# RuihanGao/visual-tactile-synthesis

Hardware: AMD Instinct MI355X
Metric: train_images_per_sec (higher is better)
Workload: dtype f32; 1 GPU; skitG G+D1+D2 train step, 1024x1024 sketch->(RGB,tactile), 4 images/GPU, 64 tactile patches/image, LPIPS/CLIP terms off (no weights offline); global_batch=4, parallelism=dp1, losses_finite=True, hip_graph=True, d2_visualisation_pass=True, train_only=False, full=False

## Files before the change

visual-tactile-synthesis_amd/csrc/vts_conv_head.hip:

```cpp
#include <limits.h>
#include <stdlib.h>

#include "vts_internal.h"

namespace {

struct HeadK {
  const float* x;
  const float *sc, *sh;
  int64_t ns;
  int C, IH, IW, OH, OW, pad, padx;
  const float* w;
  int ws_ci;
  const float* bias;
  float* out;
  int64_t ons;
  float slope;
  const float* ident;
};

constexpr int HK_TY = 32, HK_TX = 32, HK_PR = HK_TY + 3, HK_PC = HK_TX + 3, HK_PCP = 36;
constexpr int HK_MAXC = 512;

template <int CK>
__global__ __launch_bounds__(1024) void conv_head_kernel(const HeadK p) {
  constexpr int BLOCK = 1024, NG = BLOCK / 256, CPG = CK / NG;
  static_assert(CK % NG == 0, "a chunk splits evenly over the thread groups");
  constexpr int NEL = CK * HK_PR * HK_PC;
  constexpr int NLD = (NEL + BLOCK - 1) / BLOCK;
  __shared__ __attribute__((aligned(16))) float tile[CK][HK_PR][HK_PCP];
  __shared__ __attribute__((aligned(16))) float wl[CK][16];
  __shared__ float ssc[HK_MAXC], ssh[HK_MAXC];
  const int tid = threadIdx.x, n = blockIdx.z;
  const int grp = __builtin_amdgcn_readfirstlane(tid >> 8), t256 = tid & 255;
  const int tx4 = t256 & 7, ty = t256 >> 3;
  const int oy0 = blockIdx.y * HK_TY, ox0 = blockIdx.x * HK_TX;
  const int iy0 = oy0 - p.pad, ix0 = ox0 - p.padx;
  for (int c = tid; c < p.C; c += BLOCK) {
    ssc[c] = p.sc ? p.sc[n * p.C + c] : 1.f;
    ssh[c] = p.sh ? p.sh[n * p.C + c] : 0.f;
  }
  int soff[NLD], sdst[NLD];
  const int64_t plane = (int64_t)p.IH * p.IW;
#pragma unroll
  for (int i = 0; i < NLD; ++i) {
    const int e = i * BLOCK + tid;
    const int c = e / (HK_PR * HK_PC), rem = e - c * (HK_PR * HK_PC);
    const int r = rem / HK_PC, col = rem - r * HK_PC;
    const int iy = iy0 + r, ix = ix0 + col;
    const bool in = e < NEL && iy >= 0 && iy < p.IH && ix >= 0 && ix < p.IW;
    soff[i] = in ? iy * p.IW + ix : -1;
    sdst[i] = e < NEL ? (c * HK_PR + r) * HK_PCP + col : -1;
  }
  const float* xb = p.x + n * p.ns;
  float pv[NLD];
  static_assert(BLOCK <= HK_PR * HK_PC, "one boundary per slot");
  auto chan = [&](int i) {
    const int b = (i * BLOCK) / (HK_PR * HK_PC);
    return b + (tid >= (b + 1) * (HK_PR * HK_PC) - i * BLOCK ? 1 : 0);
  };
  auto load_chunk = [&](int c0) {
#pragma unroll
    for (int i = 0; i < NLD; ++i) {
      const int c = c0 + chan(i);
      pv[i] = (soff[i] >= 0 && c < p.C) ? xb[c * plane + soff[i]] : 0.f;
    }
  };
  auto store_chunk = [&](int c0) {
    float* t = &tile[0][0][0];
#pragma unroll
    for (int i = 0; i < NLD; ++i) {
      const int c = c0 + chan(i);
      if (sdst[i] >= 0) {
        const bool ok = soff[i] >= 0 && c < p.C;
        const int cc = min(c, p.C - 1);
        const float u = fmaf(pv[i], ssc[cc], ssh[cc]);
        t[sdst[i]] = ok ? fmaxf(u, 0.f) + p.slope * fminf(u, 0.f) : 0.f;
      }
    }
    if (tid < CK * 16) {
      const int c = c0 + (tid >> 4);
      wl[tid >> 4][tid & 15] = c < p.C ? p.w[(int64_t)c * p.ws_ci + (tid & 15)] : 0.f;
    }
  };
  float acc[4] = {0.f, 0.f, 0.f, 0.f};
  __syncthreads();
  load_chunk(0);
  store_chunk(0);
  __syncthreads();
  for (int c0 = 0; c0 < p.C; c0 += CK) {
    const bool more = c0 + CK < p.C;
    if (more) load_chunk(c0 + CK);
#pragma unroll
    for (int cg = 0; cg < CPG; ++cg) {
      const int c = grp * CPG + cg;
#pragma unroll
      for (int ky = 0; ky < 4; ++ky) {
        const f32x4 a = *reinterpret_cast<const f32x4*>(&tile[c][ty + ky][tx4 * 4]);
        const f32x4 b = *reinterpret_cast<const f32x4*>(&tile[c][ty + ky][tx4 * 4 + 4]);
        const f32x4 wv = *reinterpret_cast<const f32x4*>(&wl[c][ky * 4]);
        const float v[8] = {a[0], a[1], a[2], a[3], b[0], b[1], b[2], b[3]};
#pragma unroll
        for (int kx = 0; kx < 4; ++kx)
#pragma unroll
          for (int j = 0; j < 4; ++j) acc[j] = fmaf(v[j + kx], wv[kx], acc[j]);
      }
    }
    __syncthreads();
    if (more) {
      store_chunk(c0 + CK);
      __syncthreads();
    }
  }
  f32x4* red = reinterpret_cast<f32x4*>(&tile[0][0][0]);
  if (grp > 0) red[(grp - 1) * 256 + t256] = (f32x4){acc[0], acc[1], acc[2], acc[3]};
  __syncthreads();
  if (grp > 0) return;
#pragma unroll
  for (int g = 1; g < NG; ++g) {
    const f32x4 v = red[(g - 1) * 256 + t256];
#pragma unroll
    for (int j = 0; j < 4; ++j) acc[j] += v[j];
  }
  const float bias = p.bias ? p.bias[0] : 0.f;
  const int y = oy0 + ty;
  if (y < p.OH) {
    float* o = p.out + n * p.ons + (int64_t)y * p.OW;
#pragma unroll
    for (int j = 0; j < 4; ++j) {
      const int x = ox0 + tx4 * 4 + j;
      if (x < p.OW) o[x] = acc[j] + bias;
    }
  }
}

struct HeadSK {
  const float* x;
  const float *sc, *sh;
  int64_t ns;
  int C, N, IH, IW, OH, OW, pad, padx;
  const float* w;
  int ws_ci;
  const float* bias;
  float* out;
  int64_t ons;
  float slope;
  int IPB, PH, PW, CK;
};

__global__ __launch_bounds__(256) void conv_head_small_kernel(const HeadSK p) {
  extern __shared__ __attribute__((aligned(16))) float smem[];
  float* tile = smem;
  float* wl = smem + p.IPB * p.CK * p.PH * p.PW;
  const int tid = threadIdx.x;
  const int n0 = blockIdx.x * p.IPB;
  const int nimg = min(p.IPB, p.N - n0);
  const int plane = p.PH * p.PW, ohw = p.OH * p.OW, ihw = p.IH * p.IW;
  const int img = tid / ohw, r = tid - img * ohw;
  const int oy = r / p.OW, ox = r - oy * p.OW;
  const bool active = img < nimg;
  const int base = img * p.CK * plane + oy * p.PW + ox;
  for (int i = tid; i < p.IPB * p.CK * plane; i += 256) tile[i] = 0.f;
  float acc = 0.f;
  for (int c0 = 0; c0 < p.C; c0 += p.CK) {
    __syncthreads();
    const int total = nimg * p.CK * ihw;
    for (int e0 = tid; e0 < total; e0 += 256 * 8) {
      float raw[8], fsc[8], fsh[8];
      int dst[8];
#pragma unroll
      for (int j = 0; j < 8; ++j) {
        const int e = e0 + j * 256;
        const int ee = min(e, total - 1);
        const int ic = ee / ihw, q = ee - ic * ihw;
        const int im = ic / p.CK, c = ic - im * p.CK;
        const int y = q / p.IW, x = q - y * p.IW;
        const int cc = min(c0 + c, p.C - 1), n = n0 + im;
        raw[j] = p.x[n * p.ns + (int64_t)cc * ihw + q];
        fsc[j] = p.sc ? p.sc[n * p.C + cc] : 1.f;
        fsh[j] = p.sh ? p.sh[n * p.C + cc] : 0.f;
        dst[j] = (e < total && c0 + c < p.C) ? (im * p.CK + c) * plane + (y + p.pad) * p.PW + x + p.padx : -1 - ((im * p.CK + c) * plane + (y + p.pad) * p.PW + x + p.padx);
        if (e >= total) dst[j] = INT_MIN;
      }
#pragma unroll
      for (int j = 0; j < 8; ++j) {
        const float t = fmaf(raw[j], fsc[j], fsh[j]);
        if (dst[j] >= 0) tile[dst[j]] = fmaxf(t, 0.f) + p.slope * fminf(t, 0.f);
        else if (dst[j] != INT_MIN) tile[-1 - dst[j]] = 0.f;
      }
    }
    for (int e = tid; e < p.CK * 16; e += 256) wl[e] = (c0 + (e >> 4) < p.C) ? p.w[(int64_t)(c0 + (e >> 4)) * p.ws_ci + (e & 15)] : 0.f;
    __syncthreads();
    if (active) {
#pragma unroll 4
      for (int c = 0; c < p.CK; ++c) {
        const float* t = tile + base + c * plane;
#pragma unroll
        for (int ky = 0; ky < 4; ++ky)
#pragma unroll
          for (int kx = 0; kx < 4; ++kx) acc = fmaf(t[ky * p.PW + kx], wl[c * 16 + ky * 4 + kx], acc);
      }
    }
  }
  if (active) p.out[(n0 + img) * p.ons + r] = acc + (p.bias ? p.bias[0] : 0.f);
}

}

int vts_conv_head_try(const vts_conv_desc* d, hipStream_t st) {
  if (d->transposed || d->stride != 1 || d->Cout != 1 || d->in1.data || d->dmask.data || d->accumulate || d->act_out != VTS_ACT_NONE)
    return VTS_ERR_UNSUPPORTED;
  if (d->in0.C > HK_MAXC || d->in0.C < 8 || (int64_t)d->IH * d->IW * d->in0.C >= (1ll << 31)) return VTS_ERR_UNSUPPORTED;
  if ((int64_t)d->OH * d->OW < 1024) {
    const int padx = d->pad + d->pad_dx;
    if (d->N < 32 || d->OH * d->OW > 256 || d->pad < 0 || padx < 0 || d->IH + d->pad < d->OH + 3 - d->pad || d->IW + padx < d->OW + 3 - padx)
      return VTS_ERR_UNSUPPORTED;
    HeadSK q;
    q.x = d->in0.data; q.sc = d->in0.scale; q.sh = d->in0.shift; q.ns = d->in0.nstride; q.C = d->in0.C; q.N = d->N;
    q.IH = d->IH; q.IW = d->IW; q.OH = d->OH; q.OW = d->OW; q.pad = d->pad; q.padx = padx;
    q.w = d->w; q.ws_ci = d->ws_ci; q.bias = d->bias; q.out = d->out; q.ons = d->out_nstride; q.slope = vts_slope(d->act_in);
    q.PH = d->IH + 2 * d->pad; q.PW = d->IW + 2 * padx;
    q.IPB = 256 / (d->OH * d->OW);
    q.CK = d->in0.C;
    auto bytes = [&]() { return (int64_t)(q.IPB * q.CK * q.PH * q.PW + q.CK * 16) * 4; };
    while (q.IPB > 2 && bytes() > 60 * 1024) --q.IPB;
    if (bytes() > 60 * 1024) {
      q.CK = 16;
      q.IPB = 256 / (d->OH * d->OW);
      while (q.IPB > 1 && bytes() > 60 * 1024) --q.IPB;
    }
    const int lds = (int)bytes();
    if (lds > 64 * 1024) return VTS_ERR_UNSUPPORTED;
    hipLaunchKernelGGL(conv_head_small_kernel, dim3(cdiv(d->N, q.IPB)), dim3(256), lds, st, q);
    vts_set_kernel("conv_head_small_kernel");
    VTS_CHECK_LAUNCH("vts_conv4x4 (head, small maps)");
    return VTS_OK;
  }
  HeadK k;
  k.x = d->in0.data; k.sc = d->in0.scale; k.sh = d->in0.shift; k.ns = d->in0.nstride; k.C = d->in0.C;
  k.IH = d->IH; k.IW = d->IW; k.OH = d->OH; k.OW = d->OW; k.pad = d->pad; k.padx = d->pad + d->pad_dx;
  k.w = d->w; k.ws_ci = d->ws_ci; k.bias = d->bias; k.out = d->out; k.ons = d->out_nstride;
  k.slope = vts_slope(d->act_in);
  k.ident = nullptr;
  dim3 grid(cdiv(d->OW, HK_TX), cdiv(d->OH, HK_TY), d->N);
  hipLaunchKernelGGL((conv_head_kernel<8>), grid, dim3(1024), 0, st, k);
  vts_set_kernel("conv_head_kernel<8>");
  VTS_CHECK_LAUNCH("vts_conv4x4 (head)");
  return VTS_OK;
}
```

visual-tactile-synthesis_amd/csrc/vts_wgrad.hip:

```cpp
#include <stdio.h>
#include <stdlib.h>

#include "vts_internal.h"

namespace {

struct Src {
  const float *d0, *d1, *sc0, *sh0, *sc1, *sh1;
  int64_t ns0, ns1;
  int C0, C1, C;
  int act;
  float slope;
  const float* ident;
  int plain;
};

struct WgK {
  Src lo, hi;
  int N, LH, LW, HH, HW, pad, padx;
  int cl_groups, ch_groups;
  int tiles_y, tiles_x, ntiles;
  float* part;
  int ablate;
};
// ... 672 lines not shown
          for (int t = 0; t < CLT; ++t)
#pragma unroll
            for (int c = 0; c < CHW; ++c) acc[t][c] = __builtin_amdgcn_mfma_f32_16x16x4f32(a[u][t], b[u][c], acc[t][c], 0, 0, 0);
        }
      }
    }
    __syncthreads();
  }
  float* part = p.part + (int64_t)blockIdx.x * p.CL * p.CH * 16;
#pragma unroll
  for (int t = 0; t < CLT; ++t)
#pragma unroll
    for (int c = 0; c < CHW; ++c) {
      const int ch = wave * CHW + c;
#pragma unroll
      for (int r = 0; r < 4; ++r) {
        const int cl = t * 16 + kq * 4 + r;
        if (cl < p.CL && ch < p.CH) part[((int64_t)cl * p.CH + ch) * 16 + m16] = acc[t][c][r];
      }
    }
}

struct HeadWK {
  const float* lo;
  int64_t lons;
  const float *hi, *hisc, *hish;
  int64_t hins;
  int CH, N, LH, LW, HH, HW, pad, padx;
  float hi_slope;
  int tiles_y, tiles_x;
  float* part;
};
constexpr int HWG_TY = 16, HWG_TX = 32, HWG_PR = HWG_TY + 3, HWG_PC = HWG_TX + 3, HWG_PCP = 36, HWG_CK = 16, HWG_PLANE = HWG_PR * HWG_PCP;

__global__ __launch_bounds__(256) void wgrad_head_kernel(const HeadWK p) {
  __shared__ __attribute__((aligned(16))) float patch[HWG_CK * HWG_PLANE];
  __shared__ __attribute__((aligned(16))) float dyt[HWG_TY * HWG_PCP];
  const int tid = threadIdx.x;
  const int tile = blockIdx.x;
  const int n = tile / (p.tiles_y * p.tiles_x), rem = tile - n * (p.tiles_y * p.tiles_x);
  const int ty = rem / p.tiles_x, tx = rem - ty * p.tiles_x;
  const int y0 = ty * HWG_TY, x0 = tx * HWG_TX;
  const int hy0 = y0 - p.pad, hx0 = x0 - p.padx;
  for (int e = tid; e < HWG_TY * HWG_TX; e += 256) {
    const int r = e >> 5, c = e & 31;
    const int y = y0 + r, x = x0 + c;
    dyt[r * HWG_PCP + c] = (y < p.LH && x < p.LW) ? p.lo[n * p.lons + (int64_t)y * p.LW + x] : 0.f;
  }
  const int rg = tid & 3, ky = (tid >> 2) & 3, chl = tid >> 4;
  const int64_t hplane = (int64_t)p.HH * p.HW;
  float* part = p.part + (int64_t)tile * p.CH * 16;
  const int lane = tid & 63;
  const int wv = __builtin_amdgcn_readfirstlane(tid >> 6);
  const int ix = hx0 + lane;
  const bool colok = lane < HWG_PC && ix >= 0 && ix < p.HW;
  const int ixc = min(max(ix, 0), p.HW - 1);
  float raw[HWG_CK / 4][HWG_PR];
  auto load_chunk = [&](int c0) {
#pragma unroll
    for (int cc = 0; cc < HWG_CK / 4; ++cc) {
      const int chc = min(c0 + wv + 4 * cc, p.CH - 1);
      const float* src = p.hi + n * p.hins + chc * hplane + ixc;
#pragma unroll
      for (int r = 0; r < HWG_PR; ++r) raw[cc][r] = src[(int64_t)min(max(hy0 + r, 0), p.HH - 1) * p.HW];
    }
  };
  auto store_chunk = [&](int c0) {
#pragma unroll
    for (int cc = 0; cc < HWG_CK / 4; ++cc) {
      const int c = wv + 4 * cc, ch = c0 + c;
      const bool chok = ch < p.CH;
      const int chc = chok ? ch : p.CH - 1;
      const float sc = p.hisc ? p.hisc[n * p.CH + chc] : 1.f, sh = p.hish ? p.hish[n * p.CH + chc] : 0.f;
      float* dstp = patch + c * HWG_PLANE + min(lane, HWG_PCP - 1);
#pragma unroll
      for (int r = 0; r < HWG_PR; ++r) {
        const int iy = hy0 + r;
        const bool ok = chok && colok && iy >= 0 && iy < p.HH;
        const float t = fmaf(raw[cc][r], sc, sh);
        if (lane < HWG_PCP) dstp[r * HWG_PCP] = ok ? fmaxf(t, 0.f) + p.hi_slope * fminf(t, 0.f) : 0.f;
      }
    }
  };
  load_chunk(0);
  for (int c0 = 0; c0 < p.CH; c0 += HWG_CK) {
    __syncthreads();
    store_chunk(c0);
    if (c0 + HWG_CK < p.CH) load_chunk(c0 + HWG_CK);
    __syncthreads();
    float acc[4] = {0.f, 0.f, 0.f, 0.f};
#pragma unroll
    for (int j = 0; j < HWG_TY / 4; ++j) {
      const int r = rg + 4 * j;
      const f32x4* vp = reinterpret_cast<const f32x4*>(patch + chl * HWG_PLANE + (r + ky) * HWG_PCP);
      const f32x4* dp = reinterpret_cast<const f32x4*>(dyt + r * HWG_PCP);
      float v[HWG_PCP], d[HWG_TX];
#pragma unroll
      for (int i = 0; i < HWG_PCP / 4; ++i) {
        const f32x4 t = vp[i];
        v[4 * i] = t[0]; v[4 * i + 1] = t[1]; v[4 * i + 2] = t[2]; v[4 * i + 3] = t[3];
      }
#pragma unroll
      for (int i = 0; i < HWG_TX / 4; ++i) {
        const f32x4 t = dp[i];
        d[4 * i] = t[0]; d[4 * i + 1] = t[1]; d[4 * i + 2] = t[2]; d[4 * i + 3] = t[3];
      }
#pragma unroll
      for (int x = 0; x < HWG_TX; ++x)
#pragma unroll
        for (int kx = 0; kx < 4; ++kx) acc[kx] = fmaf(d[x], v[x + kx], acc[kx]);
    }
#pragma unroll
    for (int kx = 0; kx < 4; ++kx) {
      const float a = acc[kx] + __shfl_xor(acc[kx], 1);
      acc[kx] = a + __shfl_xor(a, 2);
    }
    if (rg == 0 && c0 + chl < p.CH) *reinterpret_cast<f32x4*>(part + (c0 + chl) * 16 + ky * 4) = (f32x4){acc[0], acc[1], acc[2], acc[3]};
  }
}

__global__ __launch_bounds__(1024) void wgrad_reduce_kernel(const float* __restrict__ part, int64_t n, int pw, float* __restrict__ dw,
                                                            int accumulate) {
  __shared__ float red[16][64];
  const int lane = threadIdx.x & 63, w = threadIdx.x >> 6;
  const int64_t i = (int64_t)blockIdx.x * 64 + lane;
  float s = 0.f;
  if (i < n)
    for (int k = w; k < pw; k += 16) s += part[(int64_t)k * n + i];
  red[w][lane] = s;
  __syncthreads();
  if (w == 0 && i < n) {
    float t = 0.f;
#pragma unroll
    for (int k = 0; k < 16; ++k) t += red[k][lane];
    dw[i] = accumulate ? dw[i] + t : t;
  }
}

constexpr int RB_JOBS = 40;
struct ReduceTable {
  int njobs;
  int blk_start[RB_JOBS + 1];
  unsigned char narrow[RB_JOBS];
  vts_reduce_job job[RB_JOBS];
};

constexpr int RB_ELEMS = 256;
__global__ __launch_bounds__(1024) void wgrad_reduce_batch_kernel(const ReduceTable t) {
  __shared__ f32x4 red[16][64];
  int lo = 0, hi = t.njobs - 1;
  while (lo < hi) {
    const int mid = (lo + hi + 1) >> 1;
    if (t.blk_start[mid] <= (int)blockIdx.x) lo = mid;
    else hi = mid - 1;
  }
  const vts_reduce_job& j = t.job[lo];
  const int lane = threadIdx.x & 63, w = threadIdx.x >> 6;
  if (t.narrow[lo]) {
    const int el = lane & 15, cg = lane >> 4;
    const int64_t nb = (int64_t)(blockIdx.x - t.blk_start[lo]) * 64;
    f32x4 sn = {0.f, 0.f, 0.f, 0.f};
    for (int sg = 0; sg < j.nseg; ++sg) {
      const float* part = j.part[sg];
      const int pw = j.pw[sg];
      const bool vec = nb + 64 <= j.nel && (j.nel & 3) == 0 && (reinterpret_cast<uintptr_t>(part) & 15) == 0;
      f32x4 a[8];
#pragma unroll
      for (int u = 0; u < 8; ++u) a[u] = (f32x4){0.f, 0.f, 0.f, 0.f};
      for (int k = w * 4 + cg; k < pw; k += 512) {
#pragma unroll
        for (int u = 0; u < 8; ++u) {
          const int kk = k + 64 * u;
          if (kk < pw) {
            const float* row = part + (int64_t)kk * j.nel + nb;
            f32x4 v;
            if (vec) {
              v = *reinterpret_cast<const f32x4*>(row + el * 4);
            } else {
#pragma unroll
              for (int e = 0; e < 4; ++e) v[e] = (nb + el * 4 + e < j.nel) ? row[el * 4 + e] : 0.f;
            }
            a[u] += v;
          }
        }
      }
      sn += ((a[0] + a[1]) + (a[2] + a[3])) + ((a[4] + a[5]) + (a[6] + a[7]));
    }
    f32x4 o;
#pragma unroll
    for (int e = 0; e < 4; ++e) {
      const float p1 = sn[e] + __shfl_xor(sn[e], 16);
      o[e] = p1 + __shfl_xor(p1, 32);
    }
    if (cg == 0) red[w][el] = o;
    __syncthreads();
    if (w == 0 && lane < 16) {
      f32x4 v = red[0][lane];
#pragma unroll
      for (int k = 1; k < 16; ++k) v += red[k][lane];
#pragma unroll
      for (int e = 0; e < 4; ++e) {
        const int64_t i = nb + lane * 4 + e;
        if (i < j.nel) j.dw[i] = j.accumulate ? j.dw[i] + v[e] : v[e];
      }
    }
    return;
  }
  const int64_t base = (int64_t)(blockIdx.x - t.blk_start[lo]) * RB_ELEMS;
  const bool tail = base + RB_ELEMS > j.nel;
  f32x4 s = {0.f, 0.f, 0.f, 0.f};
  for (int sg = 0; sg < j.nseg; ++sg) {
    const float* part = j.part[sg];
    const int pw = j.pw[sg];
    const bool vec = !tail && (j.nel & 3) == 0 && (reinterpret_cast<uintptr_t>(part) & 15) == 0;
    f32x4 a[8];
#pragma unroll
    for (int u = 0; u < 8; ++u) a[u] = (f32x4){0.f, 0.f, 0.f, 0.f};
    for (int k = w; k < pw; k += 128) {
#pragma unroll
      for (int u = 0; u < 8; ++u) {
        const int kk = k + 16 * u;
        if (kk < pw) {
          const float* row = part + (int64_t)kk * j.nel + base;
          f32x4 v;
          if (vec) {
            v = *reinterpret_cast<const f32x4*>(row + lane * 4);
          } else {
#pragma unroll
            for (int e = 0; e < 4; ++e) v[e] = (base + lane * 4 + e < j.nel) ? row[lane * 4 + e] : 0.f;
          }
          a[u] += v;
        }
      }
    }
    s += ((a[0] + a[1]) + (a[2] + a[3])) + ((a[4] + a[5]) + (a[6] + a[7]));
  }
  red[w][lane] = s;
  __syncthreads();
  if (w == 0) {
    f32x4 v = red[0][lane];
// ... 201 lines not shown
#undef TALL_CASE
    return false;
  }
#define NS_CASE(CLT, CHT) \
  if (pl.clt == CLT && pl.cht == CHT) { launch_ns<S, CLT, CHT>(k, pl, st); return true; }
#define NS_ROW(CLT) NS_CASE(CLT, 1) NS_CASE(CLT, 2) NS_CASE(CLT, 3) NS_CASE(CLT, 4) NS_CASE(CLT, 5)
  NS_ROW(1) NS_ROW(2) NS_ROW(3) NS_ROW(4) NS_ROW(5)
#undef NS_ROW
#undef NS_CASE
  return false;
}

}


extern "C" int64_t vts_wgrad4x4_ws_floats(const vts_wgrad_desc* d) {
  if (!d) return 0;
  const int64_t CL = d->lo0.C + (d->lo1.data ? d->lo1.C : 0), CH = d->hi0.C + (d->hi1.data ? d->hi1.C : 0);
  const Plan pl = make_plan(d);
  return (int64_t)pl.pw * CL * CH * 16;
}

extern "C" int vts_wgrad4x4(const vts_wgrad_desc* d, float* ws, void* stream) {
  VTS_CHECK_ARG(d && d->lo0.data && d->hi0.data && d->dw && ws, "vts_wgrad4x4: null pointer");
  VTS_CHECK_ARG(d->stride == 1 || d->stride == 2, "vts_wgrad4x4: stride %d unsupported", d->stride);
  VTS_CHECK_ARG(d->LH <= d->HH + 16 && d->LW <= d->HW + 16 && d->pad >= -8 && d->pad <= 8,
                "vts_wgrad4x4: lo %dx%d / pad %d implausible for hi %dx%d s%d", d->LH, d->LW, d->pad, d->HH, d->HW, d->stride);
  const Plan pl = make_plan(d);
  WgK k;
  fill_src(k.lo, d->lo0, d->lo1, d->act_lo);
  fill_src(k.hi, d->hi0, d->hi1, d->act_hi);
  k.N = d->N; k.LH = d->LH; k.LW = d->LW; k.HH = d->HH; k.HW = d->HW; k.pad = d->pad; k.padx = d->pad + d->pad_dx;
  k.cl_groups = pl.cl_groups; k.ch_groups = pl.ch_groups;
  k.tiles_y = pl.tiles_y; k.tiles_x = pl.tiles_x; k.ntiles = pl.ntiles;
  k.part = ws;
  static const int ablate = vts_tune("VTS_ABLATE", 0);
  k.ablate = ablate;
  hipStream_t st = (hipStream_t)stream;
  const int64_t nel = (int64_t)k.lo.C * k.hi.C * 16;
  if (pl.small) {
    SmallWK q;
    q.lo = d->lo0.data; q.losc = d->lo0.scale; q.losh = d->lo0.shift; q.lons = d->lo0.nstride;
    q.hi = d->hi0.data; q.hisc = d->hi0.scale; q.hish = d->hi0.shift; q.hins = d->hi0.nstride;
    q.CL = k.lo.C; q.CH = k.hi.C; q.N = d->N; q.LH = d->LH; q.LW = d->LW; q.HH = d->HH; q.HW = d->HW; q.S = d->stride; q.pad = d->pad;
    q.padx = d->pad + d->pad_dx;
    q.lo_slope = vts_slope(d->act_lo); q.hi_slope = vts_slope(d->act_hi);
    q.IPB = pl.ipb; q.nblocks = pl.nblocks; q.POS = pl.pos; q.POSP = pl.posp; q.PW_ = pl.pwf; q.PLANE = pl.plane;
    q.part = ws;
    const int64_t lob = (int64_t)d->N * d->lo0.nstride * 4, hib = (int64_t)d->N * d->hi0.nstride * 4;
    q.quads = d->lo0.nstride == (int64_t)q.CL * d->LH * d->LW && d->hi0.nstride == (int64_t)q.CH * d->HH * d->HW && lob < 0x40000000 && hib < 0x40000000;
    q.lobytes = q.quads ? (int)lob : 0; q.hibytes = q.quads ? (int)hib : 0;
    bool ok = false;
#define SW_CASE(CLT, CHW)                                                                                                      \
  if (pl.clt == CLT && pl.cht == CHW) {                                                                                        \
    const void* fn = q.quads ? (const void*)wgrad_small_kernel<CLT, CHW, true> : (const void*)wgrad_small_kernel<CLT, CHW, false>; \
    static bool attr[2] = {false, false};                                                                                      \
    if (!attr[q.quads]) {                                                                                                      \
      (void)hipFuncSetAttribute(fn, hipFuncAttributeMaxDynamicSharedMemorySize, 160 * 1024);                                   \
      attr[q.quads] = true;                                                                                                    \
    }                                                                                                                          \
    if (q.quads) hipLaunchKernelGGL((wgrad_small_kernel<CLT, CHW, true>), dim3(pl.pw), dim3(256), pl.lds_bytes, st, q);        \
    else hipLaunchKernelGGL((wgrad_small_kernel<CLT, CHW, false>), dim3(pl.pw), dim3(256), pl.lds_bytes, st, q);               \
    vts_set_kernel("wgrad_small_kernel<%d, %d>%s", CLT, CHW, q.quads ? "+quad" : "");                                          \
    ok = true;                                                                                                                 \
  }
    SW_CASE(1, 2) SW_CASE(1, 4) SW_CASE(1, 8) SW_CASE(1, 16) SW_CASE(2, 2) SW_CASE(2, 4) SW_CASE(2, 8) SW_CASE(2, 16) SW_CASE(4, 2) SW_CASE(4, 4)
    SW_CASE(4, 8)
#undef SW_CASE
    VTS_CHECK_ARG(ok, "vts_wgrad4x4: no small-map instance for clt %d chw %d", pl.clt, pl.cht);
    VTS_CHECK_LAUNCH("vts_wgrad4x4 (small maps)");
    if (d->defer) return VTS_OK;
    hipLaunchKernelGGL(wgrad_reduce_kernel, dim3((unsigned)cdiv64(nel, 64)), dim3(1024), 0, st, ws, nel, pl.pw, d->dw, d->accumulate);
    VTS_CHECK_LAUNCH("vts_wgrad4x4 reduce");
    return VTS_OK;
  }
  if (pl.head) {
    HeadWK q;
    q.lo = d->lo0.data; q.lons = d->lo0.nstride;
    q.hi = d->hi0.data; q.hisc = d->hi0.scale; q.hish = d->hi0.shift; q.hins = d->hi0.nstride;
    q.CH = k.hi.C; q.N = d->N; q.LH = d->LH; q.LW = d->LW; q.HH = d->HH; q.HW = d->HW; q.pad = d->pad; q.padx = d->pad + d->pad_dx;
    q.hi_slope = vts_slope(d->act_hi);
    q.tiles_y = pl.tiles_y; q.tiles_x = pl.tiles_x;
    q.part = ws;
    hipLaunchKernelGGL(wgrad_head_kernel, dim3(pl.ntiles), dim3(256), 0, st, q);
    vts_set_kernel("wgrad_head_kernel");
    VTS_CHECK_LAUNCH("vts_wgrad4x4 (single channel)");
    if (d->defer) return VTS_OK;
    hipLaunchKernelGGL(wgrad_reduce_kernel, dim3((unsigned)cdiv64(nel, 64)), dim3(1024), 0, st, ws, nel, pl.pw, d->dw, d->accumulate);
    VTS_CHECK_LAUNCH("vts_wgrad4x4 reduce");
    return VTS_OK;
  }
  if (pl.ns) {
    const bool ok = d->stride == 2 ? dispatch_ns<2>(k, pl, st) : dispatch_ns<1>(k, pl, st);
    VTS_CHECK_ARG(ok, "vts_wgrad4x4: no N-split instance for clt %d cht %d", pl.clt, pl.cht);
    VTS_CHECK_LAUNCH("vts_wgrad4x4 (N-split)");
    if (d->defer) return VTS_OK;
    hipLaunchKernelGGL(wgrad_reduce_kernel, dim3((unsigned)cdiv64(nel, 64)), dim3(1024), 0, st, ws, nel, pl.pw, d->dw, d->accumulate);
    VTS_CHECK_LAUNCH("vts_wgrad4x4 reduce");
    return VTS_OK;
  }
#define WG_CASE(S, CLT, CHT) \
  if (d->stride == S && pl.clt == CLT && pl.cht == CHT) launch_wg<S, CLT, CHT>(k, pl, st);
  WG_CASE(2, 1, 4) WG_CASE(2, 1, 10) WG_CASE(2, 2, 4) WG_CASE(2, 2, 10) WG_CASE(2, 3, 4) WG_CASE(2, 3, 10) WG_CASE(2, 5, 4)
  WG_CASE(1, 1, 4) WG_CASE(1, 1, 10) WG_CASE(1, 2, 4) WG_CASE(1, 2, 10) WG_CASE(1, 3, 4) WG_CASE(1, 3, 10) WG_CASE(1, 5, 4)
#undef WG_CASE
  VTS_CHECK_LAUNCH("vts_wgrad4x4");
  if (d->defer) return VTS_OK;
  hipLaunchKernelGGL(wgrad_reduce_kernel, dim3((unsigned)cdiv64(nel, 64)), dim3(1024), 0, st, ws, nel, pl.pw, d->dw,
                     d->accumulate);
  VTS_CHECK_LAUNCH("vts_wgrad4x4 reduce");
  return VTS_OK;
}

extern "C" int vts_wgrad_reduce_batch(const vts_reduce_job* jobs, int njobs, void* stream) {
  VTS_CHECK_ARG(jobs && njobs >= 0, "vts_wgrad_reduce_batch: null pointer");
  hipStream_t st = (hipStream_t)stream;
  for (int j0 = 0; j0 < njobs; j0 += RB_JOBS) {
    ReduceTable t;
    t.njobs = njobs - j0 < RB_JOBS ? njobs - j0 : RB_JOBS;
    int blocks = 0;
    for (int j = 0; j < t.njobs; ++j) {
      const vts_reduce_job& q = jobs[j0 + j];
      VTS_CHECK_ARG(q.dw && q.nel > 0 && q.nseg >= 1 && q.nseg <= VTS_REDUCE_MAX_SEG, "vts_wgrad_reduce_batch: bad job %d", j0 + j);
      for (int sg = 0; sg < q.nseg; ++sg) VTS_CHECK_ARG(q.part[sg] && q.pw[sg] >= 1, "vts_wgrad_reduce_batch: bad segment %d of job %d", sg, j0 + j);
      t.job[j] = q;
      t.blk_start[j] = blocks;
      int maxpw = 0;
      for (int sg = 0; sg < q.nseg; ++sg) maxpw = q.pw[sg] > maxpw ? q.pw[sg] : maxpw;
      constexpr int narrow_min = 256;
      t.narrow[j] = maxpw > narrow_min ? 1 : 0;
      blocks += (int)cdiv64(q.nel, t.narrow[j] ? 64 : RB_ELEMS);
    }
    t.blk_start[t.njobs] = blocks;
    hipLaunchKernelGGL(wgrad_reduce_batch_kernel, dim3((unsigned)blocks), dim3(1024), 0, st, t);
    VTS_CHECK_LAUNCH("vts_wgrad_reduce_batch");
  }
  return VTS_OK;
}
```

visual-tactile-synthesis_amd/vts/ops.py:

```python
import ctypes as C
import math
import os
from . import tune

import torch

from . import lib as L


class Act:

    __slots__ = ("data", "scale", "shift", "mean", "rstd", "padded")

    def __init__(self, data, scale=None, shift=None, mean=None, rstd=None):
        self.data, self.scale, self.shift, self.mean, self.rstd = data, scale, shift, mean, rstd
        self.padded = None

    @property
    def shape(self):
        return self.data.shape

    def operand(self):
        return L.operand(self.data, self.scale, self.shift)


TIMER = None


DETAIL = None


KNOCKOUT = tuple(k for k in tune.get("VTS_KNOCKOUT", "").split(",") if k)


def _run(label, nbytes, flops, fn, *args):
    global DETAIL
    if KNOCKOUT and label.startswith(KNOCKOUT):
        return
    if TIMER is None:
        L.check(fn(*args), label)
        return
    e0, e1 = torch.cuda.Event(enable_timing=True), torch.cuda.Event(enable_timing=True)
    e0.record()
    rc = fn(*args)
    e1.record()
    L.check(rc, label)
    if label.startswith(("conv4x4", "wgrad4x4", "patch_conv4x4", "patch_wgrad4x4", "norm_", "conv3x3_wide", "wgrad3x3_wide")):
        label = L.load().vts_last_kernel().decode()
    TIMER.append((label, nbytes, flops, e0, e1, DETAIL))
    DETAIL = None


def _numel(op):
    return 0


_ws = {}


def workspace(nfloats, device):
    key = (str(device), WS_LANE)
    t = _ws.get(key)
    if t is None or t.numel() < nfloats:
        if t is not None and frozen_ws():
            _retired.append(t)
        t = torch.empty(max(int(nfloats), 2 * (t.numel() if t is not None else 0), 1 << 20), dtype=torch.float32, device=device)
        _ws[key] = t
    return t


_retired = []

_counters = {}
FUSE_FINALIZE = tune.get("VTS_FUSE_FINALIZE", "0") == "1"


def counters(device):
    if not FUSE_FINALIZE:
        return None
    key = (str(device), WS_LANE)
    t = _counters.get(key)
    if t is None:
        t = _counters[key] = torch.zeros(1 << 16, dtype=torch.int32, device=device)
    return t


_WS_HOLDERS = set()


def freeze_ws(owner):
    _WS_HOLDERS.add(owner)


def release_ws(owner):
    _WS_HOLDERS.discard(owner)


def frozen_ws():
    return bool(_WS_HOLDERS)


WS_LANE = 0


def _op(a):
    if a is None:
        return L.Operand(None, None, None, 0, 0)
    if isinstance(a, Act):
        return a.operand()
    if isinstance(a, L.Operand):
        return a
    return L.operand(a)


BWD_SUMS = tune.get("VTS_BWD_SUMS", "1") != "0"
BSUMS = {}

_stat_ws = {}


def stat_workspace(nfloats, device):
    key = (str(device), WS_LANE)
    t = _stat_ws.get(key)
    if t is None or t.numel() < nfloats:
        if t is not None and frozen_ws():
            _retired.append(t)
        t = _stat_ws[key] = torch.empty(max(int(nfloats), 2 * (t.numel() if t is not None else 0), 1 << 18), dtype=torch.float32, device=device)
    return t


def conv4x4(in0, w, ws_co, ws_ci, cout, out, *, in1=None, bias=None, stride=2, pad=1, transposed=False, act_in=0,
            act_out=0, dmask=None, dmask_act=0, accumulate=False, out_nstride=None, in_hw=None, pad_dx=0, instance_norm=False,
            batch_norm=None, bwd_sums=False):
    lib = L.load()
    d = L.ConvDesc()
    d.in0, d.in1 = _op(in0), _op(in1)
    x = in0.data if isinstance(in0, Act) else in0
    d.N = x.shape[0]
    d.IH, d.IW = in_hw if in_hw else (x.shape[2], x.shape[3])
    d.OH, d.OW = out.shape[2], out.shape[3]
    d.Cout = cout
    d.stride, d.pad, d.transposed = stride, pad, int(transposed)
    d.pad_dx = pad_dx
    d.w, d.ws_co, d.ws_ci = w.data_ptr(), ws_co, ws_ci
    d.bias = L.ptr(bias)
    d.out = out.data_ptr()
    d.out_nstride = out.stride(0) if out_nstride is None else out_nstride
    d.act_in, d.act_out = act_in, act_out
    d.dmask = _op(dmask)
    d.dmask_act = dmask_act
    d.accumulate = int(accumulate)
    if d.OH * d.OW <= 64 * 64:
        need = lib.vts_conv4x4_ws_floats(C.byref(d))
        ws = workspace(need, x.device)
        d.ws, d.ws_floats = ws.data_ptr(), ws.numel()
    cin = d.in0.C + d.in1.C
    taps = 4 if (transposed and stride == 2) else 16
    flops = 2.0 * d.N * d.OH * d.OW * cout * cin * taps
    nbytes = 4.0 * (d.N * cin * d.IH * d.IW + d.N * cout * d.OH * d.OW * (1 + (dmask is not None) + bool(accumulate))
                    + cout * cin * 16)
    label = "conv4x4<%s,s%d,nr%d>" % ("convT" if transposed else "conv", stride, (cout + 15) // 16)
    if d.N >= 128 and max(d.IH, d.IW, d.OH, d.OW) <= 34:
        label = "patch_" + label
    if TIMER is not None:
        global DETAIL
        DETAIL = "N%d %dx%dx%d -> %dx%dx%d p%d%s%s" % (d.N, cin, d.IH, d.IW, cout, d.OH, d.OW, pad, " dmask" if dmask is not None else "",
                                                      " acc" if accumulate else "")
    if bwd_sums and dmask is not None and BWD_SUMS:
        part = torch.empty(int(lib.vts_conv4x4_norm_ws_floats(C.byref(d))), dtype=torch.float32, device=x.device)
        slots = C.c_int(-1 if bwd_sums == "in" else 0)
        _run(label, nbytes, flops, lib.vts_conv4x4_bsums, C.byref(d), part.data_ptr(), part.numel(), C.byref(slots), L.stream())
        if slots.value == -1:
            BSUMS[out.data_ptr()] = (None, -1, out)
        elif slots.value:
            BSUMS[out.data_ptr()] = (part, slots.value, out)
        else:
            BSUMS.pop(out.data_ptr(), None)
        return out
    if not instance_norm and batch_norm is None:
        BSUMS.pop(out.data_ptr(), None)
        _run(label, nbytes, flops, lib.vts_conv4x4, C.byref(d), L.stream())
        return out
    kw = dict(batch_norm) if batch_norm is not None else {}
    mode = 1 if batch_norm is not None else 0
    nd, st = _norm_desc(out, mode, **kw)
    sws = stat_workspace(lib.vts_conv4x4_norm_ws_floats(C.byref(d)), x.device)
    fused = C.c_int(0)
    _run(label, nbytes, flops, lib.vts_conv4x4_norm, C.byref(d), C.byref(nd), sws.data_ptr(), sws.numel(), C.byref(fused), L.stream())
    if fused.value >= 2:
        if TIMER is not None:
            DETAIL = "%s N%d %dx%dx%d from %d epilogue slots" % ("BN" if mode else "IN", out.shape[0], cout, d.OH, d.OW, fused.value - 2)
        _run("norm_from_partials", 12.0 * out.shape[0] * cout * (fused.value - 2), 0.0, lib.vts_norm_stats_from_partials, C.byref(nd), sws.data_ptr(), fused.value - 2, L.stream())
        return Act(out, st[0], st[1], st[2], st[3])
    if fused.value:
        return Act(out, st[0], st[1], st[2], st[3])
    return norm_stats(out, mode, **kw)


_DEFER_DEPTH = 0
_pending = []
_pending_by_dw = {}
_arenas = {}


class _Arena:

    def __init__(self, device):
        self.device, self.blocks, self.cur, self.off = device, [], 0, 0

    def alloc(self, nfloats):
        nfloats = (int(nfloats) + 63) // 64 * 64
        while True:
            if self.cur < len(self.blocks):
                b = self.blocks[self.cur]
                if self.off + nfloats <= b.numel():
                    t = b[self.off:self.off + nfloats]
                    self.off += nfloats
                    return t
                if self.off == 0:
                    _retired.append(b)
                    self.blocks[self.cur] = torch.empty(max(nfloats, 2 * b.numel()), dtype=torch.float32, device=self.device)
                    continue
                self.cur, self.off = self.cur + 1, 0
            else:
                self.blocks.append(torch.empty(max(nfloats, 16 << 20), dtype=torch.float32, device=self.device))

    def reset(self):
        self.cur, self.off = 0, 0


def _arena(device):
    key = (str(device), WS_LANE)
    a = _arenas.get(key)
    if a is None:
        a = _arenas[key] = _Arena(device)
    return a


FLUSH_BYTES = 96 << 20


def wgrad_flush(lane=None):
    global _pending
    todo = [q for q in _pending if lane is None or q["lane"] == lane]
    if not todo:
        return
    jobs = (L.ReduceJob * len(todo))()
    nbytes = 0.0
    for j, q in zip(jobs, todo):
        j.dw, j.nel, j.accumulate, j.nseg = q["dw"].data_ptr(), q["nel"], int(q["accumulate"]), len(q["segs"])
        for i, (part, pw) in enumerate(q["segs"]):
            j.part[i], j.pw[i] = part.data_ptr(), pw
            nbytes += 4.0 * pw * q["nel"]
        _pending_by_dw.pop(q["dw"].data_ptr(), None)
    if TIMER is not None:
        global DETAIL
        DETAIL = "%d jobs %.1f MB partials, copies per job %d..%d" % (len(todo), nbytes / 1e6, min(pw for q in todo for _, pw in q["segs"]),
                                                                     max(pw for q in todo for _, pw in q["segs"]))
    _run("wgrad_reduce_batch", nbytes, 0.0, L.load().vts_wgrad_reduce_batch, jobs, len(todo), L.stream())
    _pending = [q for q in _pending if not (lane is None or q["lane"] == lane)]
    for (dev, ln), a in _arenas.items():
        if lane is None or ln == lane:
            a.reset()


def wgrad_discard():
    global _pending
    _pending = []
    _pending_by_dw.clear()
    BSUMS.clear()
    for a in _arenas.values():
        a.reset()


def wgrad_pending_bytes(lane):
    return sum(4.0 * pw * q["nel"] for q in _pending if q["lane"] == lane for _, pw in q["segs"])


class deferred_wgrad:
    def __enter__(self):
        global _DEFER_DEPTH
        _DEFER_DEPTH += 1
        return self

    def __exit__(self, exc_type, exc, tb):
        global _DEFER_DEPTH
        _DEFER_DEPTH -= 1
        if _DEFER_DEPTH == 0:
            if exc_type is None:
                wgrad_flush()
            else:
                wgrad_discard()
        return False


def wgrad4x4(lo0, hi0, dw, *, lo1=None, hi1=None, act_lo=0, act_hi=0, stride=2, pad=1, accumulate=False, pad_dx=0, defer=None):
    lib = L.load()
    d = L.WgradDesc()
    d.lo0, d.lo1, d.hi0, d.hi1 = _op(lo0), _op(lo1), _op(hi0), _op(hi1)
    d.act_lo, d.act_hi = act_lo, act_hi
    lo = lo0.data if isinstance(lo0, Act) else lo0
    hi = hi0.data if isinstance(hi0, Act) else hi0
    d.N, d.LH, d.LW, d.HH, d.HW = lo.shape[0], lo.shape[2], lo.shape[3], hi.shape[2], hi.shape[3]
    d.stride, d.pad = stride, pad
    d.pad_dx = pad_dx
    d.dw = dw.data_ptr()
    d.accumulate = int(accumulate)
    n = lib.vts_wgrad4x4_ws_floats(C.byref(d))
    cl, chn = d.lo0.C + d.lo1.C, d.hi0.C + d.hi1.C
    nel = cl * chn * 16
    if defer is None:
        defer = _DEFER_DEPTH > 0
    prev = _pending_by_dw.get(dw.data_ptr()) if defer else None
    if prev is not None and (len(prev["segs"]) >= 4 or prev["nel"] != nel):
        raise RuntimeError("wgrad4x4: more than 4 deferred contributions to one weight gradient")
    ws = _arena(lo.device).alloc(n) if defer else workspace(n, lo.device)
    d.defer = int(bool(defer))
    flops = 2.0 * d.N * d.LH * d.LW * cl * chn * 16
    nbytes = 4.0 * (d.N * cl * d.LH * d.LW + d.N * chn * d.HH * d.HW + cl * chn * 16)
    if TIMER is not None:
        global DETAIL
        DETAIL = "N%d lo %dx%dx%d hi %dx%dx%d p%d" % (d.N, cl, d.LH, d.LW, chn, d.HH, d.HW, pad)
    _run(("patch_wgrad4x4<s%d>" if (d.N >= 128 and max(d.HH, d.HW) <= 34) else "wgrad4x4<s%d>") % stride, nbytes, flops, lib.vts_wgrad4x4,
         C.byref(d), ws.data_ptr(), L.stream())
    if defer:
        seg = (ws, int(n // nel))
        if prev is not None:
            assert accumulate, "a second deferred contribution to a weight gradient must accumulate"
            prev["segs"].append(seg)
        else:
            q = dict(dw=dw, nel=nel, accumulate=accumulate, segs=[seg], lane=WS_LANE)
            _pending.append(q)
            _pending_by_dw[dw.data_ptr()] = q
        if wgrad_pending_bytes(WS_LANE) > FLUSH_BYTES:
            wgrad_flush(WS_LANE)
    return dw


def _tap_blocks(K):
    nb = (K + 3) // 4
    return [(a, b) for a in range(nb) for b in range(nb)]


def tap_embed(w, K, a, b, w4):
    _run("tap_embed", 0.0, 0.0, L.load().vts_tap_embed, w.data_ptr(), w.numel() // (K * K), K, a, b, w4.data_ptr(), L.stream())
    return w4


def tap_extract(dw4, K, a, b, dw, accumulate=False):
    _run("tap_extract", 0.0, 0.0, L.load().vts_tap_extract, dw4.data_ptr(), dw.numel() // (K * K), K, a, b, dw.data_ptr(),
         int(accumulate), L.stream())
    return dw


def _w4_scratch(w, K, tag):
    key = ("w4", w.data_ptr(), tuple(w.shape), tag)
    buf = _ws.get(key)
    if buf is None:
        buf = _ws[key] = torch.zeros(len(_tap_blocks(K)), w.shape[0], w.shape[1], 4, 4, dtype=torch.float32, device=w.device)
    return buf


def convk(x, w, out, *, bias=None, pad=0, act_in=0):
    co, ci, K, _ = w.shape
    w4 = _w4_scratch(w, K, "fwd")
    for i, (a, b) in enumerate(_tap_blocks(K)):
        tap_embed(w, K, a, b, w4[i])
        conv4x4(x, w4[i], ci * 16, 16, co, out, bias=bias if i == 0 else None, stride=1, pad=pad - 4 * a, pad_dx=4 * (a - b),
                act_in=act_in, accumulate=i > 0)
    return out


def convk_bwd_data(dout, w, din, *, pad=0, accumulate=False):
    co, ci, K, _ = w.shape
    w4 = _w4_scratch(w, K, "fwd")
    for i, (a, b) in enumerate(_tap_blocks(K)):
        tap_embed(w, K, a, b, w4[i])
        conv4x4(dout, w4[i], 16, ci * 16, ci, din, stride=1, pad=pad - 4 * a, pad_dx=4 * (a - b), transposed=True,
                accumulate=accumulate or i > 0)
    return din


def wgradk(dout, x, dw, *, pad=0, act_hi=0, accumulate=False):
    co, ci, K, _ = dw.shape
    dw4 = _w4_scratch(dw, K, "grad")
    for i, (a, b) in enumerate(_tap_blocks(K)):
        wgrad4x4(dout, x, dw4[i], stride=1, pad=pad - 4 * a, pad_dx=4 * (a - b), act_hi=act_hi, defer=False)
        tap_extract(dw4[i], K, a, b, dw, accumulate=accumulate)
    return dw


def _s2_origin(K, h, w):
    oh, ow = (h - K) // 2 + 1, (w - K) // 2 + 1
    for o in range(0, 5 - K):
        if (h + 2 * o - 4) // 2 + 1 == oh and (w + 2 * o - 4) // 2 + 1 == ow:
            return o
    raise ValueError("no 4x4 embedding for a stride-2 %dx%d convolution on a %dx%d input" % (K, K, h, w))


def _embed_at(w, K, o, tag):
    w4 = _w4_scratch(w, K, tag)[0]
    _run("tap_embed", 0.0, 0.0, L.load().vts_tap_embed_at, w.data_ptr(), w.numel() // (K * K), K, -o, -o, w4.data_ptr(), L.stream())
    return w4


def convk_s2(x, w, out, *, bias=None, act_in=0):
# ... 1407 lines not shown
```

Measured before the change: 783.3 images/s.

## Rewrite conv head as register-streaming kernel, split wgrad head channels, add few-partial reduce

The single-output-channel 4x4 conv head is replaced. Instead of a 1024-thread LDS-tiled kernel, 256-thread blocks now stream input rows through registers with buffer loads and DPP lane shifts, and double-buffer channel rounds. The wgrad head kernel gets a second grid dimension over channel chunks instead of looping over all channels in one block. The batched wgrad reduction gains a specialised path for jobs with few partial rows. The profiler labels for head kernels are also adjusted. Together these aim to raise occupancy and cut LDS traffic and synchronisation in the head convolutions and reductions, at the cost of more complex code and redundant halo loads across channel waves.

```diff
diff --git a/visual-tactile-synthesis_amd/csrc/vts_conv_head.hip b/visual-tactile-synthesis_amd/csrc/vts_conv_head.hip
--- a/visual-tactile-synthesis_amd/csrc/vts_conv_head.hip
+++ b/visual-tactile-synthesis_amd/csrc/vts_conv_head.hip
@@ -19,118 +19,115 @@
   const float* ident;
 };
 
-constexpr int HK_TY = 32, HK_TX = 32, HK_PR = HK_TY + 3, HK_PC = HK_TX + 3, HK_PCP = 36;
 constexpr int HK_MAXC = 512;
-
-template <int CK>
-__global__ __launch_bounds__(1024) void conv_head_kernel(const HeadK p) {
-  constexpr int BLOCK = 1024, NG = BLOCK / 256, CPG = CK / NG;
-  static_assert(CK % NG == 0, "a chunk splits evenly over the thread groups");
-  constexpr int NEL = CK * HK_PR * HK_PC;
-  constexpr int NLD = (NEL + BLOCK - 1) / BLOCK;
-  __shared__ __attribute__((aligned(16))) float tile[CK][HK_PR][HK_PCP];
-  __shared__ __attribute__((aligned(16))) float wl[CK][16];
-  __shared__ float ssc[HK_MAXC], ssh[HK_MAXC];
-  const int tid = threadIdx.x, n = blockIdx.z;
-  const int grp = __builtin_amdgcn_readfirstlane(tid >> 8), t256 = tid & 255;
-  const int tx4 = t256 & 7, ty = t256 >> 3;
-  const int oy0 = blockIdx.y * HK_TY, ox0 = blockIdx.x * HK_TX;
-  const int iy0 = oy0 - p.pad, ix0 = ox0 - p.padx;
-  for (int c = tid; c < p.C; c += BLOCK) {
-    ssc[c] = p.sc ? p.sc[n * p.C + c] : 1.f;
-    ssh[c] = p.sh ? p.sh[n * p.C + c] : 0.f;
-  }
-  int soff[NLD], sdst[NLD];
-  const int64_t plane = (int64_t)p.IH * p.IW;
-#pragma unroll
-  for (int i = 0; i < NLD; ++i) {
-    const int e = i * BLOCK + tid;
-    const int c = e / (HK_PR * HK_PC), rem = e - c * (HK_PR * HK_PC);
-    const int r = rem / HK_PC, col = rem - r * HK_PC;
-    const int iy = iy0 + r, ix = ix0 + col;
-    const bool in = e < NEL && iy >= 0 && iy < p.IH && ix >= 0 && ix < p.IW;
-    soff[i] = in ? iy * p.IW + ix : -1;
-    sdst[i] = e < NEL ? (c * HK_PR + r) * HK_PCP + col : -1;
-  }
+constexpr int HK_T = 4;
+constexpr int HK_CU = 4;
+constexpr int HK_VL = 61;
+
+typedef __amdgpu_buffer_rsrc_t rsrc_t;
+__device__ __forceinline__ float ld_buf(const rsrc_t& rs, unsigned voff, unsigned soff) {
+  return __builtin_bit_cast(float, __builtin_amdgcn_raw_buffer_load_b32(rs, (int)voff, (int)soff, 0));
+}
+__device__ __forceinline__ float and_bits(float v, unsigned m) { return __builtin_bit_cast(float, __builtin_bit_cast(unsigned, v) & m); }
+__device__ __forceinline__ float from_next(float v) {
+  return __builtin_bit_cast(float, __builtin_amdgcn_update_dpp(0, __builtin_bit_cast(int, v), 0x130, 0xF, 0xF, true));
+}
+
+template <int T, int CU>
+__global__ __launch_bounds__(256) void conv_head_kernel(const HeadK p) {
+  constexpr int R = T + 3;
+  static_assert(T % 4 == 0, "the four waves split the rows of the final combination");
+  __shared__ float red[4][T][64];
+  const int tid = threadIdx.x, lane = tid & 63, n = blockIdx.z;
+  const int wv = __builtin_amdgcn_readfirstlane(tid >> 6);
+  const int oy0 = blockIdx.y * T, ox0 = blockIdx.x * HK_VL;
+  const int iy0 = oy0 - p.pad, ix = ox0 - p.padx + lane;
+  const unsigned cmask = (ix >= 0 && ix < p.IW) ? 0xFFFFFFFFu : 0u;
+  const unsigned vo = (unsigned)min(max(ix, 0), p.IW - 1) * 4u;
+  unsigned so[R], rmask[R];
+#pragma unroll
+  for (int r = 0; r < R; ++r) {
+    const int iy = iy0 + r;
+    so[r] = (unsigned)(min(max(iy, 0), p.IH - 1) * p.IW) * 4u;
+    rmask[r] = (iy >= 0 && iy < p.IH) ? 0xFFFFFFFFu : 0u;
+  }
+  const int plane = p.IH * p.IW;
   const float* xb = p.x + n * p.ns;
-  float pv[NLD];
-  static_assert(BLOCK <= HK_PR * HK_PC, "one boundary per slot");
-  auto chan = [&](int i) {
-    const int b = (i * BLOCK) / (HK_PR * HK_PC);
-    return b + (tid >= (b + 1) * (HK_PR * HK_PC) - i * BLOCK ? 1 : 0);
+  auto chan = [&](int j) { return (j >> 1) * 8 + wv * 2 + (j & 1); };
+  const int nch = 2 * (p.C >> 3) + min(max((p.C & 7) - 2 * wv, 0), 2);
+  const int nround = (nch + CU - 1) / CU;
+  float acc[T];
+#pragma unroll
+  for (int t = 0; t < T; ++t) acc[t] = 0.f;
+  float rawA[CU][R], rawB[CU][R];
+  auto load = [&](float (&raw)[CU][R], int round) {
+#pragma unroll
+    for (int u = 0; u < CU; ++u) {
+      const int c = min(chan(round * CU + u), p.C - 1);
+      const rsrc_t rs = __builtin_amdgcn_make_buffer_rsrc((void*)(xb + (int64_t)c * plane), 0, plane * 4, 0x00020000);
+#pragma unroll
+      for (int r = 0; r < R; ++r) raw[u][r] = ld_buf(rs, vo, so[r]);
+    }
   };
-  auto load_chunk = [&](int c0) {
-#pragma unroll
-    for (int i = 0; i < NLD; ++i) {
-      const int c = c0 + chan(i);
-      pv[i] = (soff[i] >= 0 && c < p.C) ? xb[c * plane + soff[i]] : 0.f;
-    }
+  const float* scb = p.sc ? p.sc + n * p.C : p.ident;
+  const float* shb = p.sh ? p.sh + n * p.C : p.ident + 1;
+  const int scs = p.sc ? 1 : 0, shs = p.sh ? 1 : 0;
+  float wq[16], scq, shq;
+  auto fetch_w = [&](int j) {
+    const int c = min(chan(j), p.C - 1);
+    const float* wp = p.w + (int64_t)c * p.ws_ci;
+#pragma unroll
+    for (int k = 0; k < 16; ++k) wq[k] = wp[k];
+    scq = scb[c * scs];
+    shq = shb[c * shs];
   };
-  auto store_chunk = [&](int c0) {
-    float* t = &tile[0][0][0];
-#pragma unroll
-    for (int i = 0; i < NLD; ++i) {
-      const int c = c0 + chan(i);
-      if (sdst[i] >= 0) {
-        const bool ok = soff[i] >= 0 && c < p.C;
-        const int cc = min(c, p.C - 1);
-        const float u = fmaf(pv[i], ssc[cc], ssh[cc]);
-        t[sdst[i]] = ok ? fmaxf(u, 0.f) + p.slope * fminf(u, 0.f) : 0.f;
-      }
-    }
-    if (tid < CK * 16) {
-      const int c = c0 + (tid >> 4);
-      wl[tid >> 4][tid & 15] = c < p.C ? p.w[(int64_t)c * p.ws_ci + (tid & 15)] : 0.f;
+  auto compute = [&](float (&raw)[CU][R], int round) {
+#pragma unroll
+    for (int u = 0; u < CU; ++u) {
+      const int j = round * CU + u;
+      float w[16];
+#pragma unroll
+      for (int k = 0; k < 16; ++k) w[k] = wq[k];
+      const float sc = scq, sh = shq;
+      fetch_w(j + 1);
+      if (j < nch) {
+#pragma unroll
+        for (int r = 0; r < R; ++r) {
+          const float t = fmaf(raw[u][r], sc, sh);
+          const float v0 = and_bits(fmaxf(t, 0.f) + p.slope * fminf(t, 0.f), cmask & rmask[r]);
+          const float v1 = from_next(v0), v2 = from_next(v1), v3 = from_next(v2);
+#pragma unroll
+          for (int ky = 0; ky < 4; ++ky) {
+            const int o = r - ky;
+            if (o >= 0 && o < T) {
+              acc[o] = fmaf(v0, w[ky * 4], acc[o]);
+              acc[o] = fmaf(v1, w[ky * 4 + 1], acc[o]);
+              acc[o] = fmaf(v2, w[ky * 4 + 2], acc[o]);
+              acc[o] = fmaf(v3, w[ky * 4 + 3], acc[o]);
+            }
+          }
+        }
+      }
     }
   };
-  float acc[4] = {0.f, 0.f, 0.f, 0.f};
+  fetch_w(0);
+  load(rawA, 0);
+  for (int i = 0; i < nround; i += 2) {
+    if (i + 1 < nround) load(rawB, i + 1);
+    compute(rawA, i);
+    if (i + 2 < nround) load(rawA, i + 2);
+    compute(rawB, i + 1);
+  }
+#pragma unroll
+  for (int t = 0; t < T; ++t) red[wv][t][lane] = acc[t];
   __syncthreads();
-  load_chunk(0);
-  store_chunk(0);
-  __syncthreads();
-  for (int c0 = 0; c0 < p.C; c0 += CK) {
-    const bool more = c0 + CK < p.C;
-    if (more) load_chunk(c0 + CK);
-#pragma unroll
-    for (int cg = 0; cg < CPG; ++cg) {
-      const int c = grp * CPG + cg;
-#pragma unroll
-      for (int ky = 0; ky < 4; ++ky) {
-        const f32x4 a = *reinterpret_cast<const f32x4*>(&tile[c][ty + ky][tx4 * 4]);
-        const f32x4 b = *reinterpret_cast<const f32x4*>(&tile[c][ty + ky][tx4 * 4 + 4]);
-        const f32x4 wv = *reinterpret_cast<const f32x4*>(&wl[c][ky * 4]);
-        const float v[8] = {a[0], a[1], a[2], a[3], b[0], b[1], b[2], b[3]};
-#pragma unroll
-        for (int kx = 0; kx < 4; ++kx)
-#pragma unroll
-          for (int j = 0; j < 4; ++j) acc[j] = fmaf(v[j + kx], wv[kx], acc[j]);
-      }
-    }
-    __syncthreads();
-    if (more) {
-      store_chunk(c0 + CK);
-      __syncthreads();
-    }
-  }
-  f32x4* red = reinterpret_cast<f32x4*>(&tile[0][0][0]);
-  if (grp > 0) red[(grp - 1) * 256 + t256] = (f32x4){acc[0], acc[1], acc[2], acc[3]};
-  __syncthreads();
-  if (grp > 0) return;
-#pragma unroll
-  for (int g = 1; g < NG; ++g) {
-    const f32x4 v = red[(g - 1) * 256 + t256];
-#pragma unroll
-    for (int j = 0; j < 4; ++j) acc[j] += v[j];
-  }
   const float bias = p.bias ? p.bias[0] : 0.f;
-  const int y = oy0 + ty;
-  if (y < p.OH) {
-    float* o = p.out + n * p.ons + (int64_t)y * p.OW;
-#pragma unroll
-    for (int j = 0; j < 4; ++j) {
-      const int x = ox0 + tx4 * 4 + j;
-      if (x < p.OW) o[x] = acc[j] + bias;
-    }
+  const int x = ox0 + lane;
+#pragma unroll
+  for (int j = 0; j < T / 4; ++j) {
+    const int t = wv * (T / 4) + j, y = oy0 + t;
+    const float s = ((red[0][t][lane] + red[1][t][lane]) + red[2][t][lane]) + red[3][t][lane];
+    if (lane < HK_VL && x < p.OW && y < p.OH) p.out[n * p.ons + (int64_t)y * p.OW + x] = s + bias;
   }
 }
 
@@ -241,10 +238,10 @@
   k.IH = d->IH; k.IW = d->IW; k.OH = d->OH; k.OW = d->OW; k.pad = d->pad; k.padx = d->pad + d->pad_dx;
   k.w = d->w; k.ws_ci = d->ws_ci; k.bias = d->bias; k.out = d->out; k.ons = d->out_nstride;
   k.slope = vts_slope(d->act_in);
-  k.ident = nullptr;
-  dim3 grid(cdiv(d->OW, HK_TX), cdiv(d->OH, HK_TY), d->N);
-  hipLaunchKernelGGL((conv_head_kernel<8>), grid, dim3(1024), 0, st, k);
-  vts_set_kernel("conv_head_kernel<8>");
+  k.ident = vts_ident();
+  dim3 grid(cdiv(d->OW, HK_VL), cdiv(d->OH, HK_T), d->N);
+  hipLaunchKernelGGL((conv_head_kernel<HK_T, HK_CU>), grid, dim3(256), 0, st, k);
+  vts_set_kernel("conv_head_kernel<%d, %d>", HK_T, HK_CU);
   VTS_CHECK_LAUNCH("vts_conv4x4 (head)");
   return VTS_OK;
 }
diff --git a/visual-tactile-synthesis_amd/csrc/vts_wgrad.hip b/visual-tactile-synthesis_amd/csrc/vts_wgrad.hip
--- a/visual-tactile-synthesis_amd/csrc/vts_wgrad.hip
+++ b/visual-tactile-synthesis_amd/csrc/vts_wgrad.hip
@@ -778,11 +778,11 @@
       }
     }
   };
-  load_chunk(0);
-  for (int c0 = 0; c0 < p.CH; c0 += HWG_CK) {
+  {
+    const int c0 = blockIdx.y * HWG_CK;
+    load_chunk(c0);
     __syncthreads();
     store_chunk(c0);
-    if (c0 + HWG_CK < p.CH) load_chunk(c0 + HWG_CK);
     __syncthreads();
     float acc[4] = {0.f, 0.f, 0.f, 0.f};
 #pragma unroll
@@ -842,6 +842,65 @@
 };
 
 constexpr int RB_ELEMS = 256;
+
+constexpr int RB_FEW_ELEMS = 16 * RB_ELEMS;
+template <int NU, int NW>
+__device__ __forceinline__ void reduce_few(const vts_reduce_job& j, int64_t base, int lane) {
+  constexpr int WU = (8 / NU) < NW ? (8 / NU) : NW;
+  const bool tail = base + RB_ELEMS > j.nel;
+  const f32x4 zero = {0.f, 0.f, 0.f, 0.f};
+  f32x4 total = zero;
+#pragma unroll
+  for (int w0 = 0; w0 < 16; w0 += WU) {
+    f32x4 s[WU];
+#pragma unroll
+    for (int i = 0; i < WU; ++i) s[i] = zero;
+    for (int sg = 0; sg < j.nseg; ++sg) {
+      const float* part = j.part[sg];
+      const int pw = j.pw[sg];
+      const bool vec = !tail && (j.nel & 3) == 0 && (reinterpret_cast<uintptr_t>(part) & 15) == 0;
+      f32x4 a[WU][NU];
+#pragma unroll
+      for (int i = 0; i < WU; ++i)
+#pragma unroll
+        for (int u = 0; u < NU; ++u) a[i][u] = zero;
+      if (w0 < NW && w0 < pw) {
+        f32x4 v[WU][NU];
+#pragma unroll
+        for (int i = 0; i < WU; ++i)
+#pragma unroll
+          for (int u = 0; u < NU; ++u) {
+            const int kk = min(w0 + i + 16 * u, pw - 1);
+            const float* row = part + (int64_t)kk * j.nel + base;
+            if (vec) {
+              v[i][u] = *reinterpret_cast<const f32x4*>(row + lane * 4);
+            } else {
+#pragma unroll
+              for (int e = 0; e < 4; ++e) v[i][u][e] = row[min((int64_t)(lane * 4 + e), j.nel - 1 - base)];
+            }
+          }
+#pragma unroll
+        for (int i = 0; i < WU; ++i)
+#pragma unroll
+          for (int u = 0; u < NU; ++u)
+            if (w0 + i + 16 * u < pw) a[i][u] += v[i][u];
+      }
+#pragma unroll
+      for (int i = 0; i < WU; ++i) {
+        auto A = [&](int u) { return u < NU ? a[i][u] : zero; };
+        s[i] += ((A(0) + A(1)) + (A(2) + A(3))) + ((A(4) + A(5)) + (A(6) + A(7)));
+      }
+    }
+#pragma unroll
+    for (int i = 0; i < WU; ++i) total = (w0 + i == 0) ? s[0] : total + s[i];
+  }
+#pragma unroll
+  for (int e = 0; e < 4; ++e) {
+    const int64_t i = base + lane * 4 + e;
+    if (i < j.nel) j.dw[i] = j.accumulate ? j.dw[i] + total[e] : total[e];
+  }
+}
+
 __global__ __launch_bounds__(1024) void wgrad_reduce_batch_kernel(const ReduceTable t) {
   __shared__ f32x4 red[16][64];
   int lo = 0, hi = t.njobs - 1;
@@ -852,6 +911,15 @@
   }
   const vts_reduce_job& j = t.job[lo];
   const int lane = threadIdx.x & 63, w = threadIdx.x >> 6;
+  if (t.narrow[lo] >= 2) {
+    const int64_t base = (int64_t)(blockIdx.x - t.blk_start[lo]) * RB_FEW_ELEMS + __builtin_amdgcn_readfirstlane(w) * RB_ELEMS;
+    if (base >= j.nel) return;
+    if (t.narrow[lo] == 2) reduce_few<1, 4>(j, base, lane);
+    else if (t.narrow[lo] == 3) reduce_few<1, 8>(j, base, lane);
+    else if (t.narrow[lo] == 4) reduce_few<1, 16>(j, base, lane);
+    else reduce_few<2, 16>(j, base, lane);
+    return;
+  }
   if (t.narrow[lo]) {
     const int el = lane & 15, cg = lane >> 4;
     const int64_t nb = (int64_t)(blockIdx.x - t.blk_start[lo]) * 64;
@@ -1219,7 +1287,7 @@
     q.hi_slope = vts_slope(d->act_hi);
     q.tiles_y = pl.tiles_y; q.tiles_x = pl.tiles_x;
     q.part = ws;
-    hipLaunchKernelGGL(wgrad_head_kernel, dim3(pl.ntiles), dim3(256), 0, st, q);
+    hipLaunchKernelGGL(wgrad_head_kernel, dim3(pl.ntiles, cdiv(q.CH, HWG_CK)), dim3(256), 0, st, q);
     vts_set_kernel("wgrad_head_kernel");
     VTS_CHECK_LAUNCH("vts_wgrad4x4 (single channel)");
     if (d->defer) return VTS_OK;
@@ -1266,7 +1334,8 @@
       for (int sg = 0; sg < q.nseg; ++sg) maxpw = q.pw[sg] > maxpw ? q.pw[sg] : maxpw;
       constexpr int narrow_min = 256;
       t.narrow[j] = maxpw > narrow_min ? 1 : 0;
-      blocks += (int)cdiv64(q.nel, t.narrow[j] ? 64 : RB_ELEMS);
+      if (maxpw <= 32) t.narrow[j] = maxpw <= 4 ? 2 : maxpw <= 8 ? 3 : maxpw <= 16 ? 4 : 5;
+      blocks += (int)cdiv64(q.nel, t.narrow[j] >= 2 ? RB_FEW_ELEMS : t.narrow[j] ? 64 : RB_ELEMS);
     }
     t.blk_start[t.njobs] = blocks;
     hipLaunchKernelGGL(wgrad_reduce_batch_kernel, dim3((unsigned)blocks), dim3(1024), 0, st, t);
diff --git a/visual-tactile-synthesis_amd/vts/ops.py b/visual-tactile-synthesis_amd/vts/ops.py
--- a/visual-tactile-synthesis_amd/vts/ops.py
+++ b/visual-tactile-synthesis_amd/vts/ops.py
@@ -45,7 +45,7 @@
     rc = fn(*args)
     e1.record()
     L.check(rc, label)
-    if label.startswith(("conv4x4", "wgrad4x4", "patch_conv4x4", "patch_wgrad4x4", "norm_", "conv3x3_wide", "wgrad3x3_wide")):
+    if label.startswith(("conv4x4", "wgrad4x4", "patch_conv4x4", "patch_wgrad4x4", "head_", "patch_head_", "norm_", "conv3x3_wide", "wgrad3x3_wide")):
         label = L.load().vts_last_kernel().decode()
     TIMER.append((label, nbytes, flops, e0, e1, DETAIL))
     DETAIL = None
@@ -160,6 +160,8 @@
     nbytes = 4.0 * (d.N * cin * d.IH * d.IW + d.N * cout * d.OH * d.OW * (1 + (dmask is not None) + bool(accumulate))
                     + cout * cin * 16)
     label = "conv4x4<%s,s%d,nr%d>" % ("convT" if transposed else "conv", stride, (cout + 15) // 16)
+    if cout == 1 and not transposed and stride == 1:
+        label = "head_" + label
     if d.N >= 128 and max(d.IH, d.IW, d.OH, d.OW) <= 34:
         label = "patch_" + label
     if TIMER is not None:
@@ -321,7 +323,7 @@
     if TIMER is not None:
         global DETAIL
         DETAIL = "N%d lo %dx%dx%d hi %dx%dx%d p%d" % (d.N, cl, d.LH, d.LW, chn, d.HH, d.HW, pad)
-    _run(("patch_wgrad4x4<s%d>" if (d.N >= 128 and max(d.HH, d.HW) <= 34) else "wgrad4x4<s%d>") % stride, nbytes, flops, lib.vts_wgrad4x4,
+    _run(("patch_" if (d.N >= 128 and max(d.HH, d.HW) <= 34) else "") + ("head_" if cl == 1 and stride == 1 else "") + "wgrad4x4<s%d>" % stride, nbytes, flops, lib.vts_wgrad4x4,
          C.byref(d), ws.data_ptr(), L.stream())
     if defer:
         seg = (ws, int(n // nel))
```

Measured after the change: 807.2 images/s, median of 6. 3.0% higher.
